# degleris1/CMF.jl

Hardware: NVIDIA B200
Metric: CNMF iterations/sec (higher is better)
Workload: dtype f32

## Files before the change

### cmf.jl_b200/csrc/kernels_fd.cuh

```cuda
#pragma once
#include <cuda_bf16.h>
#include <cuda_runtime.h>
#include <stdint.h>

namespace cmf {
namespace fd {

#ifndef CMF_FD_MINB
#define CMF_FD_MINB 3
#endif
constexpr int LD_U = 8;
constexpr int NT = 512;
constexpr int KQ_MAX = 128;

__device__ __forceinline__ float2 add2(float2 a, float2 b) { return __fadd2_rn(a, b); }
__device__ __forceinline__ float2 sub2(float2 a, float2 b) { return __fadd2_rn(a, make_float2(-b.x, -b.y)); }
__device__ __forceinline__ float2 mul2(float2 a, float2 b) { return __fmul2_rn(a, b); }
__device__ __forceinline__ float2 fma2(float2 a, float2 b, float2 c) { return __ffma2_rn(a, b, c); }
__device__ __forceinline__ float2 bcast(float x) { return make_float2(x, x); }

__global__ void twiddle_kernel(float2 *__restrict__ tw, int B) {
    const int m = blockIdx.x * blockDim.x + threadIdx.x;
    if (m < B) {
        float s, c;
        sincospif(-2.0f * (float)m / (float)B, &s, &c);
        tw[m] = make_float2(c, s);
    }
}
template <int B>
__device__ __forceinline__ void load_twiddles(float2 *tw, const float2 *__restrict__ twg) {
#pragma unroll
    for (int m = threadIdx.x; m < B; m += NT) tw[m] = twg[m];
}

__device__ __forceinline__ void grid_block_tile(int64_t nbx, int ny, int &blk, int &tile) {
    const unsigned dv = nbx ? (unsigned)nbx : (unsigned)ny, q = blockIdx.x / dv, r = blockIdx.x - q * dv;
    blk = (int)(nbx ? r : q);
    tile = (int)(nbx ? q : r);
}

template <int LOGB> __device__ __forceinline__ int rev(int x) { return (int)(__brev((unsigned)x) >> (32 - LOGB)); }

template <bool INV> __device__ __forceinline__ float2 twmul(float2 a, float2 w) {
    const float2 t = mul2(make_float2(a.y, a.x), INV ? make_float2(w.y, -w.y) : make_float2(-w.y, w.y));
    return fma2(a, bcast(w.x), t);
}
template <bool INV> __device__ __forceinline__ float2 mul_mi(float2 a) { return INV ? make_float2(-a.y, a.x) : make_float2(a.y, -a.x); }
template <bool INV> __device__ __forceinline__ float2 w8_sum(float2 a) {
    return INV ? add2(make_float2(a.x, a.x), make_float2(-a.y, a.y)) : add2(a, make_float2(a.y, -a.x));
}
template <bool INV> __device__ __forceinline__ float2 w83_sum(float2 a) {
    return INV ? add2(make_float2(-a.x, a.x), make_float2(-a.y, -a.y)) : add2(make_float2(a.y, -a.x), make_float2(-a.x, -a.y));
}

template <bool INV, int LOGB, int C>
__device__ __forceinline__ void fft_passes(float2 *d, const float2 *tw) {
    constexpr int B = 1 << LOGB, JSTEP = NT / C;
    const float2 rr = bcast(0.70710678118654752f);
    const int c = threadIdx.x % C, j0 = threadIdx.x / C;
#pragma unroll
    for (int s = 0; s + 2 < LOGB; s += 3) {
        const int lq = LOGB - s - 3, q = 1 << lq, qC = q * C;
#pragma unroll 1
        for (int jj = 0; jj < (B / 8 + JSTEP - 1) / JSTEP; ++jj) {
            const int j = j0 + jj * JSTEP;
            if ((B / 8) % JSTEP != 0 && j >= B / 8) break;
            const int pos = j & (q - 1), g = j >> lq;
            float2 *r = d + ((g << (lq + 3)) + pos) * C + c;
            float2 a0 = r[0], a1 = r[qC], a2 = r[2 * qC], a3 = r[3 * qC], a4 = r[4 * qC], a5 = r[5 * qC], a6 = r[6 * qC], a7 = r[7 * qC];
            float2 t, u5, v7;
            t = sub2(a0, a4); a0 = add2(a0, a4); a4 = t;
            t = sub2(a1, a5); a1 = add2(a1, a5); u5 = w8_sum<INV>(t);
            t = sub2(a2, a6); a2 = add2(a2, a6); a6 = mul_mi<INV>(t);
            t = sub2(a3, a7); a3 = add2(a3, a7); v7 = mul2(w83_sum<INV>(t), rr);
            t = sub2(a0, a2); a0 = add2(a0, a2); a2 = t;
            t = sub2(a1, a3); a1 = add2(a1, a3); a3 = mul_mi<INV>(t);
            t = sub2(a4, a6); a4 = add2(a4, a6); a6 = t;
            t = fma2(u5, rr, make_float2(-v7.x, -v7.y)); a5 = fma2(u5, rr, v7); a7 = mul_mi<INV>(t);
            t = sub2(a0, a1); a0 = add2(a0, a1); a1 = t;
            t = sub2(a2, a3); a2 = add2(a2, a3); a3 = t;
            t = sub2(a4, a5); a4 = add2(a4, a5); a5 = t;
            t = sub2(a6, a7); a6 = add2(a6, a7); a7 = t;
            if (lq > 0) {
                const int e = pos << s;
                a1 = twmul<INV>(a1, tw[4 * e]); a2 = twmul<INV>(a2, tw[2 * e]); a3 = twmul<INV>(a3, tw[6 * e]);
                a4 = twmul<INV>(a4, tw[e]);     a5 = twmul<INV>(a5, tw[5 * e]); a6 = twmul<INV>(a6, tw[3 * e]);
                a7 = twmul<INV>(a7, tw[7 * e]);
            }
            r[0] = a0; r[qC] = a1; r[2 * qC] = a2; r[3 * qC] = a3; r[4 * qC] = a4; r[5 * qC] = a5; r[6 * qC] = a6; r[7 * qC] = a7;
        }
        __syncthreads();
    }
    if constexpr (LOGB % 3 == 2) {
#pragma unroll
        for (int jj = 0; jj < (B / 4 + JSTEP - 1) / JSTEP; ++jj) {
            const int j = j0 + jj * JSTEP;
            if ((B / 4) % JSTEP != 0 && j >= B / 4) break;
            float2 *r = d + (4 * j) * C + c;
            float2 a0 = r[0], a1 = r[C], a2 = r[2 * C], a3 = r[3 * C], t;
            t = sub2(a0, a2); a0 = add2(a0, a2); a2 = t;
            t = sub2(a1, a3); a1 = add2(a1, a3); a3 = mul_mi<INV>(t);
            r[0] = add2(a0, a1); r[C] = sub2(a0, a1); r[2 * C] = add2(a2, a3); r[3 * C] = sub2(a2, a3);
        }
        __syncthreads();
    } else if constexpr (LOGB % 3 == 1) {
#pragma unroll
        for (int jj = 0; jj < (B / 2 + JSTEP - 1) / JSTEP; ++jj) {
            const int j = j0 + jj * JSTEP;
            if ((B / 2) % JSTEP != 0 && j >= B / 2) break;
            float2 *r0 = d + (2 * j) * C + c, *r1 = r0 + C;
            const float2 a = *r0, b = *r1;
            *r0 = add2(a, b);
            *r1 = sub2(a, b);
        }
        __syncthreads();
    }
}

template <int LOGB, int C>
__device__ __forceinline__ void unpack_pair(const float2 *d, int f, int p, float2 &re, float2 &im) {
    constexpr int B = 1 << LOGB;
    const float2 z = d[rev<LOGB>(f) * C + p], y = d[rev<LOGB>((B - f) & (B - 1)) * C + p];
    const float2 sm = add2(z, y), df = sub2(z, y);
    re = mul2(sm, bcast(0.5f));
    im = mul2(make_float2(df.y, df.x), make_float2(0.5f, -0.5f));
}

template <int LOGB, int C>
__device__ __forceinline__ void pack_pair(float2 *d, int f, int p, float2 re, float2 im) {
    constexpr int B = 1 << LOGB;
    if (f == 0 || f == B / 2) im = make_float2(0.f, 0.f);
    const float2 v = make_float2(im.y, im.x);
    const float2 sm = add2(re, v), df = sub2(re, v);
    d[f * C + p] = make_float2(df.x, sm.y);
    if (f > 0 && f < B / 2) d[(B - f) * C + p] = make_float2(sm.x, df.y);
}

__device__ __forceinline__ void split2(float2 ab, uint32_t &h, uint32_t &l) {
    const __nv_bfloat162 hh = __floats2bfloat162_rn(ab.x, ab.y);
    const float2 lf = sub2(ab, __bfloat1622float2(hh));
    const __nv_bfloat162 ll = __floats2bfloat162_rn(lf.x, lf.y);
    h = *reinterpret_cast<const uint32_t *>(&hh);
    l = *reinterpret_cast<const uint32_t *>(&ll);
}
__device__ __forceinline__ void store_split2(__nv_bfloat16 *hi, __nv_bfloat16 *lo, int64_t idx, float2 ab) {
    uint32_t h, l;
    split2(ab, h, l);
    *reinterpret_cast<uint32_t *>(hi + idx) = h;
    *reinterpret_cast<uint32_t *>(lo + idx) = l;
}

template <int LOGB>
__global__ void __launch_bounds__(NT, CMF_FD_MINB)
fft_x_kernel(const float *__restrict__ X, __nv_bfloat16 *__restrict__ hi, __nv_bfloat16 *__restrict__ lo, int64_t N, int64_t xcols,
             int V, int64_t nblkp, int64_t nbx, const float2 *__restrict__ twg) {
    constexpr int B = 1 << LOGB, C = 16, ISTEP = NT / C;
    extern __shared__ float2 fd_smem[];
    float2 *d = fd_smem, *tw = fd_smem + B * C;
    int b, tile;
    grid_block_tile(nbx, (int)((N + 31) / 32), b, tile);
    const int p = threadIdx.x % C;
    const int n = tile * 32 + 2 * p;
    load_twiddles<B>(tw, twg);
    {
        const int i0 = threadIdx.x / C;
        const int64_t lim64 = xcols - (int64_t)b * V;
        const int lim = (n < N) ? (int)(lim64 < 0 ? 0 : (lim64 > B ? B : lim64)) : 0;
        const float *src = X + ((int64_t)b * V + i0) * N + n;
        float2 *dst = d + i0 * C + p;
#pragma unroll 1
        for (int i = i0; i < B; i += LD_U * ISTEP, src += (int64_t)LD_U * ISTEP * N, dst += LD_U * ISTEP * C) {
            float2 v[LD_U];
#pragma unroll
            for (int u = 0; u < LD_U; ++u) {
                v[u] = make_float2(0.f, 0.f);
                if (i + u * ISTEP < lim) v[u] = *reinterpret_cast<const float2 *>(src + (int64_t)u * ISTEP * N);
            }
#pragma unroll
            for (int u = 0; u < LD_U; ++u)
                if (B % (LD_U * ISTEP) == 0 || i + u * ISTEP < B) dst[u * ISTEP * C] = v[u];
        }
    }
    __syncthreads();
    fft_passes<false, LOGB, C>(d, tw);
    if (n >= N) return;
    for (int f = threadIdx.x / C; f <= B / 2; f += NT / C) {
        float2 re, im;
        unpack_pair<LOGB, C>(d, f, p, re, im);
        const int64_t r = ((int64_t)f * nblkp + b) * 2;
        store_split2(hi, lo, r * N + n, re);
        store_split2(hi, lo, (r + 1) * N + n, im);
    }
}

template <int LOGB, int C>
__global__ void __launch_bounds__(NT, CMF_FD_MINB)
fft_h_kernel(const float *__restrict__ H, __nv_bfloat16 *__restrict__ hi, __nv_bfloat16 *__restrict__ lo, int64_t K, int64_t Tl,
             int64_t hcols, int V, int64_t nblkp, int full, int64_t t_off, int kq, int64_t nbx,
             const float2 *__restrict__ twg) {
    constexpr int B = 1 << LOGB, ISTEP = NT / C;
    const int64_t KQ = kq, MROWS = 2 * kq;
    extern __shared__ float2 fd_smem[];
    float2 *d = fd_smem, *tw = fd_smem + B * C;
    int bi, tile;
    grid_block_tile(nbx, (kq / 2) / C, bi, tile);
    const int64_t b = bi;
    const int p = threadIdx.x % C;
    const int k = 2 * (tile * C + p);
    load_twiddles<B>(tw, twg);
    {
        const int i0 = threadIdx.x / C;
        const int64_t tb = b * V + t_off;
        const int64_t lim64 = full ? (hcols - tb) : ((Tl - tb < V) ? Tl - tb : V);
        const int lim = (int)(lim64 < 0 ? 0 : (lim64 > B ? B : lim64));
        const float *src = H + (tb + i0) * K + k;
        float2 *dst = d + i0 * C + p;
        const bool pair = ((K & 1) == 0) && (k + 1 < K);
#pragma unroll 1
        for (int i = i0; i < B; i += LD_U * ISTEP, src += (int64_t)LD_U * ISTEP * K, dst += LD_U * ISTEP * C) {
            float2 v[LD_U];
#pragma unroll
            for (int u = 0; u < LD_U; ++u) {
                v[u] = make_float2(0.f, 0.f);
                if (i + u * ISTEP < lim) {
                    const float *q = src + (int64_t)u * ISTEP * K;
                    if (pair) v[u] = *reinterpret_cast<const float2 *>(q);
                    else { if (k < K) v[u].x = q[0]; if (k + 1 < K) v[u].y = q[1]; }
                }
            }
#pragma unroll
            for (int u = 0; u < LD_U; ++u)
                if (B % (LD_U * ISTEP) == 0 || i + u * ISTEP < B) dst[u * ISTEP * C] = v[u];
        }
    }
    __syncthreads();
    fft_passes<false, LOGB, C>(d, tw);
    const int64_t rs = full ? 2 * KQ : 2 * MROWS;
    const int64_t rstep = (int64_t)(NT / C) * nblkp * rs;
    int64_t r = ((int64_t)(threadIdx.x / C) * nblkp + b) * rs + k;
    for (int f = threadIdx.x / C; f <= B / 2; f += NT / C, r += rstep) {
        float2 re, im;
        unpack_pair<LOGB, C>(d, f, p, re, im);
        uint32_t hr, lr, hi_, li_;
        split2(re, hr, lr);
        split2(im, hi_, li_);
        if (full) {
            *reinterpret_cast<uint32_t *>(hi + r) = hr; *reinterpret_cast<uint32_t *>(lo + r) = lr;
            *reinterpret_cast<uint32_t *>(hi + r + KQ) = hi_; *reinterpret_cast<uint32_t *>(lo + r + KQ) = li_;
            continue;
        }
        const uint32_t sg = 0x80008000u;
        *reinterpret_cast<uint32_t *>(hi + r) = hr; *reinterpret_cast<uint32_t *>(lo + r) = lr;
        *reinterpret_cast<uint32_t *>(hi + r + KQ) = hi_ ^ sg; *reinterpret_cast<uint32_t *>(lo + r + KQ) = li_ ^ sg;
        *reinterpret_cast<uint32_t *>(hi + r + MROWS) = hi_; *reinterpret_cast<uint32_t *>(lo + r + MROWS) = li_;
        *reinterpret_cast<uint32_t *>(hi + r + MROWS + KQ) = hr; *reinterpret_cast<uint32_t *>(lo + r + MROWS + KQ) = lr;
    }
}

template <int LOGB, int C>
__global__ void __launch_bounds__(NT, CMF_FD_MINB)
fft_w_kernel(const float *__restrict__ Wi, __nv_bfloat16 *__restrict__ hi, __nv_bfloat16 *__restrict__ lo, int64_t N, int64_t K,
             int64_t L, int64_t ldw, int64_t coff, int xmode, int kq, const float2 *__restrict__ twg) {
    constexpr int B = 1 << LOGB, ISTEP = NT / C;
    const int64_t KQ = kq, MROWS = 2 * kq;
    extern __shared__ float2 fd_smem[];
    float2 *d = fd_smem, *tw = fd_smem + B * C;
    const int64_t k = blockIdx.y;
    const int p = threadIdx.x % C;
    const int64_t n = (int64_t)blockIdx.x * (2 * C) + 2 * p;
    load_twiddles<B>(tw, twg);
    {
        const int i0 = threadIdx.x / C;
        const float *src = Wi + ((int64_t)i0 * K + k) * N + n;
        float2 *dst = d + i0 * C + p;
#pragma unroll 1
        for (int i = i0; i < B; i += LD_U * ISTEP, src += (int64_t)LD_U * ISTEP * K * N, dst += LD_U * ISTEP * C) {
            float2 v[LD_U];
#pragma unroll
            for (int u = 0; u < LD_U; ++u) {
                const int ii = i + u * ISTEP;
                v[u] = make_float2(0.f, 0.f);
                if (ii < L && n < N) {
                    const float *q = src + (int64_t)u * ISTEP * K * N;
                    if ((N & 1) == 0) v[u] = *reinterpret_cast<const float2 *>(q);
                    else { v[u].x = q[0]; if (n + 1 < N) v[u].y = q[1]; }
                }
            }
#pragma unroll
            for (int u = 0; u < LD_U; ++u)
                if (B % (LD_U * ISTEP) == 0 || i + u * ISTEP < B) dst[u * ISTEP * C] = v[u];
        }
    }
    __syncthreads();
    fft_passes<false, LOGB, C>(d, tw);
    if (n >= N) return;
    for (int f = threadIdx.x / C; f <= B / 2; f += NT / C) {
        float2 re, im;
        unpack_pair<LOGB, C>(d, f, p, re, im);
        const float2 nim = make_float2(-im.x, -im.y);
        if (xmode) {
            const int64_t r0 = (((int64_t)f * 2 + 0) * MROWS + k) * N + n, r1 = r0 + MROWS * N;
            store_split2(hi, lo, r0, re);
            store_split2(hi, lo, r0 + KQ * N, nim);
            store_split2(hi, lo, r1, im);
            store_split2(hi, lo, r1 + KQ * N, re);
            continue;
        }
        const int64_t rw = ((int64_t)f * MROWS + k) * ldw + n, iw = rw + KQ * ldw;
        store_split2(hi, lo, rw, re);
        store_split2(hi, lo, rw + coff, im);
        store_split2(hi, lo, iw, nim);
        store_split2(hi, lo, iw + coff, re);
    }
}

template <int LOGB, int C>
__global__ void __launch_bounds__(NT, CMF_FD_MINB)
ifft_numH_kernel(const float *__restrict__ Of, float *__restrict__ numH, int64_t K, int64_t Tl, int V, int64_t nblkp, int kq,
                 int64_t nbx, const float2 *__restrict__ twg) {
    constexpr int B = 1 << LOGB, FSTEP = NT / C;
    const int64_t KQ = kq, MROWS = 2 * kq;
    extern __shared__ float2 fd_smem[];
    float2 *d = fd_smem, *tw = fd_smem + B * C;
    int bi, tile;
    grid_block_tile(nbx, (kq / 2) / C, bi, tile);
    const int64_t b = bi;
    const int p = threadIdx.x % C;
    const int k = 2 * (tile * C + p);
    load_twiddles<B>(tw, twg);
    {
        const int f0 = threadIdx.x / C;
        const int64_t ustep = (int64_t)FSTEP * nblkp * MROWS;
        const float *o = Of + ((int64_t)f0 * nblkp + b) * MROWS + k;
#pragma unroll 1
        for (int f = f0; f <= B / 2; f += 4 * FSTEP, o += 4 * ustep) {
            float2 re[4], im[4];
#pragma unroll
            for (int u = 0; u < 4; ++u)
                if (f + u * FSTEP <= B / 2) {
                    const float *q = o + u * ustep;
                    re[u] = *reinterpret_cast<const float2 *>(q); im[u] = *reinterpret_cast<const float2 *>(q + KQ);
                }
#pragma unroll
            for (int u = 0; u < 4; ++u)
                if (f + u * FSTEP <= B / 2) pack_pair<LOGB, C>(d, f + u * FSTEP, p, re[u], im[u]);
        }
    }
    __syncthreads();
    fft_passes<true, LOGB, C>(d, tw);
    const float2 sc = bcast(1.0f / (float)B);
    const bool pair = ((K & 1) == 0) && (k + 1 < K);
    for (int i = threadIdx.x / C; i < V; i += NT / C) {
        const int64_t t = b * V + i;
        if (t >= Tl) break;
        const float2 z = mul2(d[rev<LOGB>(i) * C + p], sc);
        if (pair) *reinterpret_cast<float2 *>(numH + t * K + k) = z;
        else { if (k < K) numH[t * K + k] = z.x; if (k + 1 < K) numH[t * K + k + 1] = z.y; }
    }
}

template <int LOGB>
__global__ void __launch_bounds__(NT, CMF_FD_MINB)
ifft_resid_kernel(const float *__restrict__ Yf, const float *__restrict__ X, double *__restrict__ partial, int64_t N, int64_t Tl,
                  int64_t L, int V, int64_t nbc, int64_t b0, int64_t nbx, const float2 *__restrict__ twg) {
    constexpr int B = 1 << LOGB, C = 16, FSTEP = NT / C, ISTEP = NT / C;
    extern __shared__ float2 fd_smem[];
    __shared__ double red[NT / 32];
    float2 *d = fd_smem, *tw = fd_smem + B * C;
    const int ny = (int)((N + 31) / 32);
    int bc, by;
    grid_block_tile(nbx, ny, bc, by);
    const int p = threadIdx.x % C;
    const int n = by * 32 + 2 * p;
    load_twiddles<B>(tw, twg);
    {
        const int f0 = threadIdx.x / C;
        const int64_t ustep = (int64_t)FSTEP * nbc * 2 * N;
        const float *y = Yf + (((int64_t)f0 * nbc + bc) * 2) * N + n;
#pragma unroll 1
        for (int f = f0; f <= B / 2; f += 4 * FSTEP, y += 4 * ustep) {
            float2 re[4], im[4];
#pragma unroll
            for (int u = 0; u < 4; ++u) {
                re[u] = make_float2(0.f, 0.f); im[u] = re[u];
                if (f + u * FSTEP <= B / 2 && n < N) {
                    const float *q = y + u * ustep;
                    re[u] = *reinterpret_cast<const float2 *>(q); im[u] = *reinterpret_cast<const float2 *>(q + N);
                }
            }
#pragma unroll
            for (int u = 0; u < 4; ++u)
                if (f + u * FSTEP <= B / 2) pack_pair<LOGB, C>(d, f + u * FSTEP, p, re[u], im[u]);
        }
    }
    __syncthreads();
    fft_passes<true, LOGB, C>(d, tw);
    const float2 sc = bcast(1.0f / (float)B);
    double accd = 0.0;
    if (n < N) {
        const int64_t tb = (b0 + bc) * (int64_t)V - (L - 1);
        const int lim = (int)(Tl - tb < B ? Tl - tb : B);
        const int i0 = (int)(L - 1) + threadIdx.x / C;
        const float *xs = X + (tb + i0) * N + n;
#pragma unroll 1
        for (int i = i0; i < B; i += LD_U * ISTEP, xs += (int64_t)LD_U * ISTEP * N) {
            float2 x[LD_U];
#pragma unroll
            for (int u = 0; u < LD_U; ++u) {
                x[u] = make_float2(0.f, 0.f);
                if (i + u * ISTEP < lim) x[u] = *reinterpret_cast<const float2 *>(xs + (int64_t)u * ISTEP * N);
            }
            float acc = 0.f;
#pragma unroll
            for (int u = 0; u < LD_U; ++u) {
                const int ii = i + u * ISTEP;
                if (ii < lim) {
                    const float2 r = fma2(d[rev<LOGB>(ii) * C + p], sc, make_float2(-x[u].x, -x[u].y));
                    acc = fmaf(r.x, r.x, acc);
                    acc = fmaf(r.y, r.y, acc);
                }
            }
            accd += (double)acc;
        }
    }
#pragma unroll
    for (int o = 16; o > 0; o >>= 1) accd += __shfl_xor_sync(0xffffffffu, accd, o);
    if ((threadIdx.x & 31) == 0) red[threadIdx.x >> 5] = accd;
    __syncthreads();
    if (threadIdx.x == 0) {
        double s = 0.0;
        for (int w = 0; w < NT / 32; ++w) s += red[w];
        partial[(int64_t)bc * ny + by] = s;
    }
}

template <typename OutT, int LOGB, int C>
__global__ void __launch_bounds__(NT, CMF_FD_MINB)
ifft_numW_kernel(const float *__restrict__ Df, OutT *__restrict__ out, int64_t N, int64_t ldi, int64_t K, int64_t L, int kq,
                 const float2 *__restrict__ twg) {
    constexpr int B = 1 << LOGB, FSTEP = NT / C;
    const int64_t KQ = kq, MROWS = 2 * kq;
    extern __shared__ float2 fd_smem[];
    float2 *d = fd_smem, *tw = fd_smem + B * C;
    const int64_t k = blockIdx.y;
    const int p = threadIdx.x % C;
    const int64_t n = (int64_t)blockIdx.x * (2 * C) + 2 * p;
    load_twiddles<B>(tw, twg);
    {
        const int f0 = threadIdx.x / C;
        const int64_t ustep = (int64_t)FSTEP * MROWS * ldi;
        const float *src = Df + ((int64_t)f0 * MROWS + k) * ldi + n;
#pragma unroll 1
        for (int f = f0; f <= B / 2; f += 4 * FSTEP, src += 4 * ustep) {
            float2 re[4], im[4];
#pragma unroll
            for (int u = 0; u < 4; ++u) {
                re[u] = make_float2(0.f, 0.f); im[u] = re[u];
                if (f + u * FSTEP <= B / 2 && n < N) {
                    re[u] = *reinterpret_cast<const float2 *>(src + u * ustep);
                    im[u] = *reinterpret_cast<const float2 *>(src + u * ustep + KQ * ldi);
                }
            }
#pragma unroll
            for (int u = 0; u < 4; ++u)
                if (f + u * FSTEP <= B / 2) pack_pair<LOGB, C>(d, f + u * FSTEP, p, re[u], im[u]);
        }
    }
    __syncthreads();
    fft_passes<true, LOGB, C>(d, tw);
    if (n >= N) return;
    const float2 sc = bcast(1.0f / (float)B);
    for (int l = threadIdx.x / C; l < L; l += NT / C) {
        const float2 z = mul2(d[rev<LOGB>(l) * C + p], sc);
        OutT *o = out + ((int64_t)l * K + k) * N + n;
        if (sizeof(OutT) == 4) {
            *reinterpret_cast<float2 *>(o) = z;
        } else {
            o[0] = (OutT)z.x;
            if (n + 1 < N) o[1] = (OutT)z.y;
        }
    }
}

}
}
```

Measured before the change: 21.80.

## Stage FFT kernel loads into shared memory via cp.async instead of registers

Replaces register-staged global loads of twiddles, X, W and Yf spectra with cp.async copies straight into shared memory, adding wait_all before each barrier. The aim is to cut register pressure and instruction overhead on the load phase and keep more bytes in flight. It also adds lane-swapped shared memory accesses for C==8 radix-2 passes and unpacking to avoid bank conflicts, and stores the partial-sum slot in shared memory. The in-place staging of the Yf pack depends on ordering between the staged reads and the pack_pair writes, which is a correctness risk.

```diff
diff --git a/cmf.jl_b200/csrc/kernels_fd.cuh b/cmf.jl_b200/csrc/kernels_fd.cuh
--- a/cmf.jl_b200/csrc/kernels_fd.cuh
+++ b/cmf.jl_b200/csrc/kernels_fd.cuh
@@ -27,10 +27,21 @@
         tw[m] = make_float2(c, s);
     }
 }
+
+__device__ __forceinline__ void cp_async4(void *dst, const void *src, bool ok) {
+    asm volatile("cp.async.ca.shared.global [%0], [%1], 4, %2;\n" ::"r"((unsigned)__cvta_generic_to_shared(dst)), "l"(src),
+                 "r"(ok ? 4 : 0) : "memory");
+}
+__device__ __forceinline__ void cp_async8(void *dst, const void *src, bool ok) {
+    asm volatile("cp.async.ca.shared.global [%0], [%1], 8, %2;\n" ::"r"((unsigned)__cvta_generic_to_shared(dst)), "l"(src),
+                 "r"(ok ? 8 : 0) : "memory");
+}
+__device__ __forceinline__ void cp_async_wait_all() { asm volatile("cp.async.wait_all;\n" ::: "memory"); }
+
 template <int B>
 __device__ __forceinline__ void load_twiddles(float2 *tw, const float2 *__restrict__ twg) {
 #pragma unroll
-    for (int m = threadIdx.x; m < B; m += NT) tw[m] = twg[m];
+    for (int m = threadIdx.x; m < B; m += NT) cp_async8(tw + m, twg + m, true);
 }
 
 __device__ __forceinline__ void grid_block_tile(int64_t nbx, int ny, int &blk, int &tile) {
@@ -109,9 +120,19 @@
             const int j = j0 + jj * JSTEP;
             if ((B / 2) % JSTEP != 0 && j >= B / 2) break;
             float2 *r0 = d + (2 * j) * C + c, *r1 = r0 + C;
-            const float2 a = *r0, b = *r1;
-            *r0 = add2(a, b);
-            *r1 = sub2(a, b);
+            if constexpr (C == 8) {
+                const bool sw = (threadIdx.x & 16) != 0;
+                float2 *pa = sw ? r1 : r0, *pb = sw ? r0 : r1;
+                const float2 u = *pa, v = *pb;
+                const float2 a = sw ? v : u, b = sw ? u : v;
+                const float2 s0 = add2(a, b), s1 = sub2(a, b);
+                *pa = sw ? s1 : s0;
+                *pb = sw ? s0 : s1;
+            } else {
+                const float2 a = *r0, b = *r1;
+                *r0 = add2(a, b);
+                *r1 = sub2(a, b);
+            }
         }
         __syncthreads();
     }
@@ -120,7 +141,17 @@
 template <int LOGB, int C>
 __device__ __forceinline__ void unpack_pair(const float2 *d, int f, int p, float2 &re, float2 &im) {
     constexpr int B = 1 << LOGB;
-    const float2 z = d[rev<LOGB>(f) * C + p], y = d[rev<LOGB>((B - f) & (B - 1)) * C + p];
+    const int rz = rev<LOGB>(f) * C + p, ry = rev<LOGB>((B - f) & (B - 1)) * C + p;
+    float2 z, y;
+    if constexpr (C == 8) {
+        const bool sw = (threadIdx.x & 16) != 0;
+        const float2 u = d[sw ? ry : rz], v = d[sw ? rz : ry];
+        z = sw ? v : u;
+        y = sw ? u : v;
+    } else {
+        z = d[rz];
+        y = d[ry];
+    }
     const float2 sm = add2(z, y), df = sub2(z, y);
     re = mul2(sm, bcast(0.5f));
     im = mul2(make_float2(df.y, df.x), make_float2(0.5f, -0.5f));
@@ -134,6 +165,19 @@
     const float2 sm = add2(re, v), df = sub2(re, v);
     d[f * C + p] = make_float2(df.x, sm.y);
     if (f > 0 && f < B / 2) d[(B - f) * C + p] = make_float2(sm.x, df.y);
+}
+
+template <int LOGB, int C>
+__device__ __forceinline__ void stage_pair(float2 *d, int f, int p, const float *re, const float *im, bool ok, const float *base) {
+    constexpr int B = 1 << LOGB;
+    cp_async8(d + f * C + p, ok ? re : base, ok);
+    if (f > 0 && f < B / 2) cp_async8(d + (B - f) * C + p, ok ? im : base, ok);
+}
+template <int LOGB, int C>
+__device__ __forceinline__ void pack_staged(float2 *d, int f, int p) {
+    constexpr int B = 1 << LOGB;
+    const float2 re = d[f * C + p], im = (f > 0 && f < B / 2) ? d[(B - f) * C + p] : make_float2(0.f, 0.f);
+    pack_pair<LOGB, C>(d, f, p, re, im);
 }
 
 __device__ __forceinline__ void split2(float2 ab, uint32_t &h, uint32_t &l) {
@@ -168,18 +212,9 @@
         const int lim = (n < N) ? (int)(lim64 < 0 ? 0 : (lim64 > B ? B : lim64)) : 0;
         const float *src = X + ((int64_t)b * V + i0) * N + n;
         float2 *dst = d + i0 * C + p;
-#pragma unroll 1
-        for (int i = i0; i < B; i += LD_U * ISTEP, src += (int64_t)LD_U * ISTEP * N, dst += LD_U * ISTEP * C) {
-            float2 v[LD_U];
-#pragma unroll
-            for (int u = 0; u < LD_U; ++u) {
-                v[u] = make_float2(0.f, 0.f);
-                if (i + u * ISTEP < lim) v[u] = *reinterpret_cast<const float2 *>(src + (int64_t)u * ISTEP * N);
-            }
-#pragma unroll
-            for (int u = 0; u < LD_U; ++u)
-                if (B % (LD_U * ISTEP) == 0 || i + u * ISTEP < B) dst[u * ISTEP * C] = v[u];
-        }
+#pragma unroll 4
+        for (int i = i0; i < B; i += ISTEP, src += (int64_t)ISTEP * N, dst += ISTEP * C) cp_async8(dst, i < lim ? src : X, i < lim);
+        cp_async_wait_all();
     }
     __syncthreads();
     fft_passes<false, LOGB, C>(d, tw);
@@ -232,6 +267,7 @@
             for (int u = 0; u < LD_U; ++u)
                 if (B % (LD_U * ISTEP) == 0 || i + u * ISTEP < B) dst[u * ISTEP * C] = v[u];
         }
+        cp_async_wait_all();
     }
     __syncthreads();
     fft_passes<false, LOGB, C>(d, tw);
@@ -273,23 +309,19 @@
         const int i0 = threadIdx.x / C;
         const float *src = Wi + ((int64_t)i0 * K + k) * N + n;
         float2 *dst = d + i0 * C + p;
-#pragma unroll 1
-        for (int i = i0; i < B; i += LD_U * ISTEP, src += (int64_t)LD_U * ISTEP * K * N, dst += LD_U * ISTEP * C) {
-            float2 v[LD_U];
-#pragma unroll
-            for (int u = 0; u < LD_U; ++u) {
-                const int ii = i + u * ISTEP;
-                v[u] = make_float2(0.f, 0.f);
-                if (ii < L && n < N) {
-                    const float *q = src + (int64_t)u * ISTEP * K * N;
-                    if ((N & 1) == 0) v[u] = *reinterpret_cast<const float2 *>(q);
-                    else { v[u].x = q[0]; if (n + 1 < N) v[u].y = q[1]; }
-                }
-            }
-#pragma unroll
-            for (int u = 0; u < LD_U; ++u)
-                if (B % (LD_U * ISTEP) == 0 || i + u * ISTEP < B) dst[u * ISTEP * C] = v[u];
-        }
+        const int lim = (n < N) ? (int)(L < B ? L : B) : 0;
+        if ((N & 1) == 0) {
+#pragma unroll 4
+            for (int i = i0; i < B; i += ISTEP, src += (int64_t)ISTEP * K * N, dst += ISTEP * C) cp_async8(dst, i < lim ? src : Wi, i < lim);
+        } else {
+#pragma unroll 4
+            for (int i = i0; i < B; i += ISTEP, src += (int64_t)ISTEP * K * N, dst += ISTEP * C) {
+                const bool oy = i < lim && n + 1 < N;
+                cp_async4(&dst->x, i < lim ? src : Wi, i < lim);
+                cp_async4(&dst->y, oy ? src + 1 : Wi, oy);
+            }
+        }
+        cp_async_wait_all();
     }
     __syncthreads();
     fft_passes<false, LOGB, C>(d, tw);
@@ -345,6 +377,7 @@
             for (int u = 0; u < 4; ++u)
                 if (f + u * FSTEP <= B / 2) pack_pair<LOGB, C>(d, f + u * FSTEP, p, re[u], im[u]);
         }
+        cp_async_wait_all();
     }
     __syncthreads();
     fft_passes<true, LOGB, C>(d, tw);
@@ -366,10 +399,12 @@
     constexpr int B = 1 << LOGB, C = 16, FSTEP = NT / C, ISTEP = NT / C;
     extern __shared__ float2 fd_smem[];
     __shared__ double red[NT / 32];
+    __shared__ int64_t slot;
     float2 *d = fd_smem, *tw = fd_smem + B * C;
     const int ny = (int)((N + 31) / 32);
     int bc, by;
     grid_block_tile(nbx, ny, bc, by);
+    if (threadIdx.x == 0) slot = (int64_t)bc * ny + by;
     const int p = threadIdx.x % C;
     const int n = by * 32 + 2 * p;
     load_twiddles<B>(tw, twg);
@@ -377,21 +412,10 @@
         const int f0 = threadIdx.x / C;
         const int64_t ustep = (int64_t)FSTEP * nbc * 2 * N;
         const float *y = Yf + (((int64_t)f0 * nbc + bc) * 2) * N + n;
-#pragma unroll 1
-        for (int f = f0; f <= B / 2; f += 4 * FSTEP, y += 4 * ustep) {
-            float2 re[4], im[4];
-#pragma unroll
-            for (int u = 0; u < 4; ++u) {
-                re[u] = make_float2(0.f, 0.f); im[u] = re[u];
-                if (f + u * FSTEP <= B / 2 && n < N) {
-                    const float *q = y + u * ustep;
-                    re[u] = *reinterpret_cast<const float2 *>(q); im[u] = *reinterpret_cast<const float2 *>(q + N);
-                }
-            }
-#pragma unroll
-            for (int u = 0; u < 4; ++u)
-                if (f + u * FSTEP <= B / 2) pack_pair<LOGB, C>(d, f + u * FSTEP, p, re[u], im[u]);
-        }
+#pragma unroll 4
+        for (int f = f0; f <= B / 2; f += FSTEP, y += ustep) stage_pair<LOGB, C>(d, f, p, y, y + N, n < N, Yf);
+        cp_async_wait_all();
+        for (int f = f0; f <= B / 2; f += FSTEP) pack_staged<LOGB, C>(d, f, p);
     }
     __syncthreads();
     fft_passes<true, LOGB, C>(d, tw);
@@ -430,7 +454,7 @@
     if (threadIdx.x == 0) {
         double s = 0.0;
         for (int w = 0; w < NT / 32; ++w) s += red[w];
-        partial[(int64_t)bc * ny + by] = s;
+        partial[slot] = s;
     }
 }
 
@@ -465,6 +489,7 @@
             for (int u = 0; u < 4; ++u)
                 if (f + u * FSTEP <= B / 2) pack_pair<LOGB, C>(d, f + u * FSTEP, p, re[u], im[u]);
         }
+        cp_async_wait_all();
     }
     __syncthreads();
     fft_passes<true, LOGB, C>(d, tw);
```

After: 22.12, median of 6. About the same (+1.5%).
